# AgentMaker/PAPC

Measured on AMD Instinct MI355X. Metric: point-clouds/sec (fwd+bwd) PointNet++SSG B=32 N=4096, higher is better.
Workload: dtype f32

## Files before the change

papc_amd/csrc/capi.hip:

```cpp
#include <stdarg.h>
#include <string.h>

#include <mutex>
#include <vector>

#include "common.h"

#define GEMM_PARTS_DEFAULT 768

namespace papc {

static thread_local char g_err[512] = "";

void set_error(const char *fmt, ...)
{
    va_list ap;
    va_start(ap, fmt);
    vsnprintf(g_err, sizeof(g_err), fmt, ap);
    va_end(ap);
}

int check_launch(const char *what)
{
    hipError_t e = hipGetLastError();
    if (e != hipSuccess) {
        set_error("%s: %s", what, hipGetErrorString(e));
        return PAPC_E_LAUNCH;
    }
    return PAPC_OK;
}

struct KnobDef { const char *name; int def, lo, hi; };
static const KnobDef g_knob_defs[KNOB_COUNT] = {
    {"PAPC_LG_PARTS", 2048, 1, 8192},
    {"PAPC_DW_F32", 0, 0, 1},
    {"PAPC_DW_DBG", 0, 0, 1},
    {"PAPC_DW_XYZ", 1, 0, 1},
    {"PAPC_PARTS", GEMM_PARTS_DEFAULT, 1, 1024},
    {"PAPC_GEMM_F32", 0, 0, 1},
    {"PAPC_GEMM_WAVES", 0, 0, 8},
    {"PAPC_MAXCAT_WAVES", 8, 4, 8},
    {"PAPC_GEMM_WS", 0, 0, 3},
    {"PAPC_GEMM_OCC", 0, 0, 1},
    {"PAPC_GEMM_DBG", 0, 0, 1},
    {"PAPC_GEMM_KB", 0, 0, 2},
    {"PAPC_GEMM_MINWG", 192, 1, 4096},
    {"PAPC_GEMM_TL", 0, 0, 1},
    {"PAPC_FPS_THREADS", 0, 0, 1024},
    {"PAPC_FPS_THREADS_SMALL", 0, 0, 1024},
    {"PAPC_STREAM", 1, 0, 1},
    {"PAPC_STREAM_MINTILES", 2048, 1, 1 << 30},
    {"PAPC_STREAM_CK", 0, 0, 8},
    {"PAPC_STREAM_ASM", 1, 0, 1},
    {"PAPC_PFN_MFMA", 1, 0, 1},
    {"PAPC_DW_RS64", 1, 0, 1},
    {"PAPC_DW_ROWS", 1, 0, 1},
    {"PAPC_DW_ROWS_BLOCKS", 4, 1, 16},
    {"PAPC_DW_ROWSX", 1, 0, 1},
    {"PAPC_PG_DBG", 0, 0, 15},
    {"PAPC_PG_NB", 0, 0, 2},
    {"PAPC_PG_NS", 0, 0, 3},
    {"PAPC_STREAM_MAXCAT", 1, 0, 1},
    {"PAPC_MAX_NOSTORE", 1, 0, 1},
    {"PAPC_PFN_FUSED_TAILS", 1, 0, 1},
    {"PAPC_STREAM_NW12", 1, 0, 1},
    {"PAPC_LG_LISTS", 1, 0, 1},
    {"PAPC_FOLD_WAVES", 16, 8, 16},
    {"PAPC_LGL_VARIANT", 0, 0, 3},
    {"PAPC_LG_PP", 1, 0, 1},
    {"PAPC_PG_GROUP", 1, 0, 1},
};
static int g_knobs[KNOB_COUNT];
static int knob_parse(int id, const char *e)
{
    const KnobDef &d = g_knob_defs[id];
    if (!e || !*e) return d.def;
    const int v = atoi(e);
    return (v < d.lo || v > d.hi) ? d.def : v;
}
static const bool g_knobs_loaded = [] {
    for (int i = 0; i < KNOB_COUNT; ++i) g_knobs[i] = knob_parse(i, getenv(g_knob_defs[i].name));
    return true;
}();
int knob(int id) { return g_knobs[id]; }

struct ProfState {
    std::mutex mu;
    unsigned mask = 0;
    std::vector<std::pair<hipEvent_t, hipEvent_t>> pending[PAPC_K_COUNT];
    std::vector<hipEvent_t> pool;
    double total_ms[PAPC_K_COUNT] = {0};
    int64_t launches[PAPC_K_COUNT] = {0};
};
static ProfState g_prof;

static hipEvent_t prof_get_event()
{
    if (!g_prof.pool.empty()) {
        hipEvent_t e = g_prof.pool.back();
        g_prof.pool.pop_back();
        return e;
    }
    hipEvent_t e;
    if (hipEventCreate(&e) != hipSuccess) return nullptr;
    return e;
}

ProfScope::ProfScope(int k, hipStream_t s) : kernel(k), stream(s), on(false), e0(nullptr)
{
    if (!(g_prof.mask & (1u << k))) return;
    std::lock_guard<std::mutex> lk(g_prof.mu);
    e0 = prof_get_event();
    if (!e0) return;
    on = hipEventRecord(e0, stream) == hipSuccess;
}

ProfScope::~ProfScope()
{
    if (!on) return;
    std::lock_guard<std::mutex> lk(g_prof.mu);
    hipEvent_t e1 = prof_get_event();
    if (!e1) return;
    if (hipEventRecord(e1, stream) == hipSuccess) g_prof.pending[kernel].push_back({e0, e1});
}

static void prof_drain(int k)
{
    for (auto &pr : g_prof.pending[k]) {
        float ms = 0.f;
        if (hipEventSynchronize(pr.second) == hipSuccess && hipEventElapsedTime(&ms, pr.first, pr.second) == hipSuccess) {
            g_prof.total_ms[k] += ms;
            g_prof.launches[k] += 1;
        }
        g_prof.pool.push_back(pr.first);
        g_prof.pool.push_back(pr.second);
    }
    g_prof.pending[k].clear();
}

}

extern "C" {

int papc_version(void) { return 600;  }

int papc_abi_version(void) { return PAPC_ABI_VERSION; }

int64_t papc_abi_sizeof(const char *struct_name)
{
    if (!struct_name) return -1;
#define PAPC_SIZEOF(T) if (strcmp(struct_name, #T) == 0) return (int64_t)sizeof(T);
    PAPC_SIZEOF(papc_group_src)
    PAPC_SIZEOF(papc_point_lists)
    PAPC_SIZEOF(papc_group_max)
    PAPC_SIZEOF(papc_bwd_dy)
    PAPC_SIZEOF(papc_scatter_dst)
    PAPC_SIZEOF(papc_bwd_red)
    PAPC_SIZEOF(papc_reduce_job)
    PAPC_SIZEOF(papc_fold_job)
    PAPC_SIZEOF(papc_fold_list)
    PAPC_SIZEOF(papc_sa_desc)
    PAPC_SIZEOF(papc_sa_layer)
    PAPC_SIZEOF(papc_compact_src)
    PAPC_SIZEOF(papc_sa_io)
    PAPC_SIZEOF(papc_sa_plan)
    PAPC_SIZEOF(papc_sa_grads)
    PAPC_SIZEOF(papc_pfn_desc)
    PAPC_SIZEOF(papc_pfn_io)
    PAPC_SIZEOF(papc_head_fc_layer)
    PAPC_SIZEOF(papc_head_bwd_job)
    PAPC_SIZEOF(papc_pg_wjob)
    PAPC_SIZEOF(papc_pg_prep)
    PAPC_SIZEOF(papc_pg_gemm)
    PAPC_SIZEOF(papc_pg_fold_job)
    PAPC_SIZEOF(papc_copy_job)
#undef PAPC_SIZEOF
    return -1;
}

const char *papc_last_error_string(void) { return papc::g_err; }

int papc_knob_set(const char *name, int value)
{
    PAPC_REQUIRE(name, PAPC_E_INVALID, "papc_knob_set: null name");
    for (int i = 0; i < papc::KNOB_COUNT; ++i)
        if (!strcmp(name, papc::g_knob_defs[i].name)) {
            PAPC_REQUIRE(value >= papc::g_knob_defs[i].lo && value <= papc::g_knob_defs[i].hi, PAPC_E_INVALID,
                         "papc_knob_set: %s = %d outside [%d, %d]", name, value, papc::g_knob_defs[i].lo, papc::g_knob_defs[i].hi);
            papc::g_knobs[i] = value;
            return PAPC_OK;
        }
    papc::set_error("papc_knob_set: unknown knob %s", name);
    return PAPC_E_INVALID;
}

int papc_knob_get(const char *name, int *value)
{
    PAPC_REQUIRE(name && value, PAPC_E_INVALID, "papc_knob_get: null argument");
    for (int i = 0; i < papc::KNOB_COUNT; ++i)
        if (!strcmp(name, papc::g_knob_defs[i].name)) { *value = papc::g_knobs[i]; return PAPC_OK; }
    papc::set_error("papc_knob_get: unknown knob %s", name);
    return PAPC_E_INVALID;
}

int papc_prof_enable(unsigned mask)
{
    std::lock_guard<std::mutex> lk(papc::g_prof.mu);
    papc::g_prof.mask = mask;
    return PAPC_OK;
}

int papc_prof_reset(void)
{
    std::lock_guard<std::mutex> lk(papc::g_prof.mu);
    for (int k = 0; k < PAPC_K_COUNT; ++k) {
        papc::prof_drain(k);
        papc::g_prof.total_ms[k] = 0;
        papc::g_prof.launches[k] = 0;
    }
    return PAPC_OK;
}

int papc_prof_read(int kernel, double *total_ms, int64_t *launches)
// ... 11 lines not shown
```

papc_amd/csrc/common.h:

```cpp
#pragma once
#include <hip/hip_runtime.h>
#include <stdint.h>
#include <stdio.h>
#include <stdlib.h>
#include <string.h>
#include <algorithm>

#include "papc_hip.h"

namespace papc {

void set_error(const char *fmt, ...);
int check_launch(const char *what);

#define PAPC_REQUIRE(cond, code, ...)      \
    do {                                   \
        if (!(cond)) {                     \
            papc::set_error(__VA_ARGS__);  \
            return (code);                 \
        }                                  \
    } while (0)

enum Knob {
    KNOB_LG_PARTS, KNOB_DW_F32, KNOB_DW_DBG, KNOB_DW_XYZ, KNOB_PARTS, KNOB_GEMM_F32, KNOB_GEMM_WAVES, KNOB_MAXCAT_WAVES,
    KNOB_GEMM_WS, KNOB_GEMM_OCC, KNOB_GEMM_DBG, KNOB_GEMM_KB, KNOB_GEMM_MINWG, KNOB_GEMM_TL, KNOB_FPS_THREADS,
    KNOB_FPS_THREADS_SMALL, KNOB_STREAM, KNOB_STREAM_MINTILES, KNOB_STREAM_CK, KNOB_STREAM_ASM, KNOB_PFN_MFMA, KNOB_DW_RS64, KNOB_DW_ROWS, KNOB_DW_ROWS_BLOCKS, KNOB_DW_ROWSX, KNOB_PG_DBG, KNOB_PG_NB, KNOB_PG_NS, KNOB_STREAM_MAXCAT, KNOB_MAX_NOSTORE, KNOB_PFN_FUSED_TAILS, KNOB_STREAM_NW12, KNOB_LG_LISTS, KNOB_FOLD_WAVES, KNOB_LGL_VARIANT, KNOB_LG_PP, KNOB_PG_GROUP, KNOB_COUNT
};
int knob(int id);

struct ProfScope {
    int kernel;
    hipStream_t stream;
    bool on;
    hipEvent_t e0;
    ProfScope(int kernel, hipStream_t stream);
    ~ProfScope();
};

static inline hipStream_t as_stream(papc_stream_t s) { return reinterpret_cast<hipStream_t>(s); }

static inline int64_t cdiv(int64_t a, int64_t b) { return (a + b - 1) / b; }
static inline bool aligned16(const void *p) { return (reinterpret_cast<uintptr_t>(p) & 15) == 0; }

#define PAPC_DPP(v, ctrl, rmask) __builtin_amdgcn_update_dpp((int)(v), (int)(v), (ctrl), (rmask), 0xF, false)

__device__ __forceinline__ float wave_sum_f32_to_lane63(float v)
{
    float t;
    t = __int_as_float(PAPC_DPP(__float_as_int(v), 0xB1, 0xF));  v += t;
    t = __int_as_float(PAPC_DPP(__float_as_int(v), 0x4E, 0xF));  v += t;
    t = __int_as_float(PAPC_DPP(__float_as_int(v), 0x124, 0xF)); v += t;
    t = __int_as_float(PAPC_DPP(__float_as_int(v), 0x128, 0xF)); v += t;
    t = __int_as_float(__builtin_amdgcn_update_dpp(0, __float_as_int(v), 0x142, 0xA, 0xF, false)); v += t;
    t = __int_as_float(__builtin_amdgcn_update_dpp(0, __float_as_int(v), 0x143, 0xC, 0xF, false)); v += t;
    return v;
}

__device__ __forceinline__ float half_sum_f32(float v)
{
    float t;
    t = __int_as_float(PAPC_DPP(__float_as_int(v), 0xB1, 0xF));  v += t;
    t = __int_as_float(PAPC_DPP(__float_as_int(v), 0x4E, 0xF));  v += t;
    t = __int_as_float(PAPC_DPP(__float_as_int(v), 0x124, 0xF)); v += t;
    t = __int_as_float(PAPC_DPP(__float_as_int(v), 0x128, 0xF)); v += t;
    t = __int_as_float(__builtin_amdgcn_update_dpp(0, __float_as_int(v), 0x142, 0xA, 0xF, false)); v += t;
    return v;
}

__device__ __forceinline__ float readlane63_f32(float v)
{
    return __int_as_float(__builtin_amdgcn_readlane(__float_as_int(v), 63));
}


#define PAPC_DPPF(v, ctrl, rmask) __int_as_float(__builtin_amdgcn_update_dpp(__float_as_int(v), __float_as_int(v), (ctrl), (rmask), 0xF, false))
#define PAPC_DPPU(v, ctrl, rmask) ((unsigned)__builtin_amdgcn_update_dpp((int)(v), (int)(v), (ctrl), (rmask), 0xF, false))

__device__ __forceinline__ float row_max_f32(float v)
{
    v = fmaxf(v, PAPC_DPPF(v, 0xB1, 0xF));
    v = fmaxf(v, PAPC_DPPF(v, 0x4E, 0xF));
    v = fmaxf(v, PAPC_DPPF(v, 0x124, 0xF));
    v = fmaxf(v, PAPC_DPPF(v, 0x128, 0xF));
    return v;
}
__device__ __forceinline__ unsigned row_min_u32(unsigned v)
{
    unsigned t;
    t = PAPC_DPPU(v, 0xB1, 0xF);  v = t < v ? t : v;
    t = PAPC_DPPU(v, 0x4E, 0xF);  v = t < v ? t : v;
    t = PAPC_DPPU(v, 0x124, 0xF); v = t < v ? t : v;
    t = PAPC_DPPU(v, 0x128, 0xF); v = t < v ? t : v;
    return v;
}
__device__ __forceinline__ float wave_max_f32_to_lane63(float v)
{
    v = row_max_f32(v);
    v = fmaxf(v, PAPC_DPPF(v, 0x142, 0xA));
    v = fmaxf(v, PAPC_DPPF(v, 0x143, 0xC));
    return v;
}
__device__ __forceinline__ unsigned wave_min_u32_to_lane63(unsigned v)
{
    unsigned t;
    v = row_min_u32(v);
    t = PAPC_DPPU(v, 0x142, 0xA); v = t < v ? t : v;
    t = PAPC_DPPU(v, 0x143, 0xC); v = t < v ? t : v;
    return v;
}
#define PAPC_DPP_STEP(op, v, ctrl) asm volatile("s_nop 1\n\t" op " %0, %0, %0 " ctrl : "+v"(v))
__device__ __forceinline__ unsigned row_max_u32_fused(unsigned v)
{
    PAPC_DPP_STEP("v_max_u32_dpp", v, "quad_perm:[1,0,3,2] row_mask:0xf bank_mask:0xf");
    PAPC_DPP_STEP("v_max_u32_dpp", v, "quad_perm:[2,3,0,1] row_mask:0xf bank_mask:0xf");
    PAPC_DPP_STEP("v_max_u32_dpp", v, "row_ror:4 row_mask:0xf bank_mask:0xf");
    PAPC_DPP_STEP("v_max_u32_dpp", v, "row_ror:8 row_mask:0xf bank_mask:0xf");
    return v;
}
__device__ __forceinline__ unsigned row_min_u32_fused(unsigned v)
{
    PAPC_DPP_STEP("v_min_u32_dpp", v, "quad_perm:[1,0,3,2] row_mask:0xf bank_mask:0xf");
    PAPC_DPP_STEP("v_min_u32_dpp", v, "quad_perm:[2,3,0,1] row_mask:0xf bank_mask:0xf");
    PAPC_DPP_STEP("v_min_u32_dpp", v, "row_ror:4 row_mask:0xf bank_mask:0xf");
    PAPC_DPP_STEP("v_min_u32_dpp", v, "row_ror:8 row_mask:0xf bank_mask:0xf");
    return v;
}
__device__ __forceinline__ unsigned wave_max_u32_fused_to_lane63(unsigned v)
{
    v = row_max_u32_fused(v);
    PAPC_DPP_STEP("v_max_u32_dpp", v, "row_bcast:15 row_mask:0xa bank_mask:0xf");
    PAPC_DPP_STEP("v_max_u32_dpp", v, "row_bcast:31 row_mask:0xc bank_mask:0xf");
    asm volatile("s_nop 1" ::"v"(v));
    return v;
}
__device__ __forceinline__ unsigned wave_min_u32_fused_to_lane63(unsigned v)
{
    v = row_min_u32_fused(v);
    PAPC_DPP_STEP("v_min_u32_dpp", v, "row_bcast:15 row_mask:0xa bank_mask:0xf");
    PAPC_DPP_STEP("v_min_u32_dpp", v, "row_bcast:31 row_mask:0xc bank_mask:0xf");
    asm volatile("s_nop 1" ::"v"(v));
    return v;
}
__device__ __forceinline__ unsigned readlane63_u32(unsigned v) { return (unsigned)__builtin_amdgcn_readlane((int)v, 63); }
__device__ __forceinline__ float readlane0_f32(float v) { return __int_as_float(__builtin_amdgcn_readlane(__float_as_int(v), 0)); }
__device__ __forceinline__ unsigned readlane0_u32(unsigned v) { return (unsigned)__builtin_amdgcn_readlane((int)v, 0); }

__device__ __forceinline__ void lds_barrier()
{
    asm volatile("s_waitcnt lgkmcnt(0)\n\ts_barrier" ::: "memory");
}

__device__ __forceinline__ float relu_np(float t) { return !(t <= 0.f) ? t : 0.f; }
__device__ __forceinline__ int lane_id() { return (int)(threadIdx.x & 63); }

}
```

papc_amd/csrc/smallm.hip:

```cpp
#include "fold.h"
#include "mlp_loaders.h"

namespace papc {

enum { PG_EPI_STORE = 0, PG_EPI_FWD = 1, PG_EPI_FWD_GMAX = 2, PG_EPI_RED = 3 };
enum { PG_PREP_PLAIN = 0, PG_PREP_CONCAT = 1, PG_PREP_BNRELU = 2, PG_PREP_DY_DENSE = 3, PG_PREP_DY_MAX = 4 };

__host__ __device__ static inline int64_t ru64(int64_t a, int64_t b) { return (a + b - 1) / b * b; }

__device__ __forceinline__ void store_planes8(char *frag0, int slot, const float (&v)[8])
{
    bf16x8 pl[3];
    split8(v, pl);
    *reinterpret_cast<uint4 *>(frag0 + slot * 16) = __builtin_bit_cast(uint4, pl[0]);
    *reinterpret_cast<uint4 *>(frag0 + 1024 + slot * 16) = __builtin_bit_cast(uint4, pl[1]);
    *reinterpret_cast<uint4 *>(frag0 + 2048 + slot * 16) = __builtin_bit_cast(uint4, pl[2]);
}

struct WJob {
    const float *src; int64_t sr, sc;
    int R, K;
    char *dst;
};
struct WJobs {
// ... 168 lines not shown
#pragma unroll
                for (int i = 0; i < 8; ++i) e[i] = dy_elem(d[i], e[i], cs[0][kl + i], cs[1][kl + i], cs[2][kl + i], cs[3][kl + i], cs[4][kl + i], cs[5][kl + i]);
            }
#pragma unroll
            for (int i = 0; i < 8; ++i) v[j][i] = (mok && kok) ? e[i] : 0.f;
        }
    }
    if (p.P) {
#pragma unroll
        for (int j = 0; j < 2; ++j) store_planes8(p.P + ((int64_t)mb * p.KBp + cb * 2 + j) * 3072, lane, v[j]);
    }
    if (p.PT) {
#pragma unroll
        for (int j = 0; j < 2; ++j)
#pragma unroll
            for (int i = 0; i < 8; ++i) tile[wv][r_in][16 * j + 8 * h + i] = v[j][i];
        __syncthreads();
#pragma unroll
        for (int j = 0; j < 2; ++j) {
            float u[8];
#pragma unroll
            for (int i = 0; i < 8; ++i) u[i] = tile[wv][16 * j + 8 * h + i][r_in];
            store_planes8(p.PT + ((int64_t)cb * p.KBt + mb * 2 + j) * 3072, lane, u);
        }
    }
}

struct PgArgs {
    const char *a, *b; int KB;
    int nst;
    int R1, R2;
    float *c; int64_t ldc, zstride;
    const float *bias;
    float *stats;
    float *gmax, *gmin; int32_t *amax, *amin;
    const float *y_prev, *mean, *invstd, *scale, *shift;
    int dbg;
    int g1, g2;
};

__device__ __forceinline__ void glds16(const char *g, unsigned lds_addr)
{
    unsigned keep;
    asm volatile("s_mov_b32 %0, m0\n\ts_mov_b32 m0, %2\n\ts_nop 0\n\tglobal_load_lds_dwordx4 %1, off\n\ts_mov_b32 m0, %0"
                 : "=&s"(keep)
                 : "v"(g), "s"(lds_addr)
                 : "memory");
}
template <int N>
__device__ __forceinline__ void pg_wait_barrier()
{
    asm volatile("s_waitcnt vmcnt(%0) lgkmcnt(0)\n\ts_barrier" ::"n"(N) : "memory");
}

template <int EPI, int NB, bool FULL>
__device__ __forceinline__ void pg_epilogue(const PgArgs &p, floatx16 (&acc)[2][NB], char *smem, int lane, int wr, int wc, int bi, int bj, int bz)
{
    const int cl = lane & 31, h = lane >> 5;
    constexpr bool FWD = (EPI == PG_EPI_FWD || EPI == PG_EPI_FWD_GMAX);
    constexpr bool SUMS = FWD || EPI == PG_EPI_RED;
    float *rs = reinterpret_cast<float *>(smem);
    if (SUMS) __syncthreads();
    const int it0 = 2 * wr * 32 + h * 4;
    const int ldc = (int)p.ldc;
#pragma unroll
    for (int ib = 0; ib < NB; ++ib) {
        const int jt = (wc * NB + ib) * 32 + cl;
        const int j = bj * (NB * 64) + jt;
        const bool jok = FULL || j < p.R2;
        const int jj = jok ? j : 0;
        float *cp = p.c + (int64_t)bz * p.zstride + (int64_t)(bi * 128 + it0) * p.ldc + jj;
        float bias = 0.f, sc = 0.f, sh = 0.f, mu = 0.f, is = 0.f;
        if (FWD && p.bias) bias = p.bias[jj];
        if (EPI == PG_EPI_RED) { sc = p.scale[jj]; sh = p.shift[jj]; mu = p.mean[jj]; is = p.invstd[jj]; }
        float yp[2][16];
        if (EPI == PG_EPI_RED) {
            const float *yq = p.y_prev + (int64_t)(bi * 128 + it0) * p.ldc + jj;
#pragma unroll
            for (int ia = 0; ia < 2; ++ia)
#pragma unroll
                for (int r = 0; r < 16; ++r) {
                    const int ro = ia * 32 + (r >> 2) * 8 + (r & 3);
                    yp[ia][r] = (FULL || (jok && bi * 128 + it0 + ro < p.R1)) ? yq[ro * ldc] : 0.f;
                }
        }
        if (FWD) {
#pragma unroll
            for (int ia = 0; ia < 2; ++ia)
#pragma unroll
                for (int r = 0; r < 16; ++r) acc[ia][ib][r] += bias;
        }
#pragma unroll
        for (int ia = 0; ia < 2; ++ia)
#pragma unroll
            for (int r = 0; r < 16; ++r) {
                const int ro = ia * 32 + (r >> 2) * 8 + (r & 3);
                if (FULL) cp[ro * ldc] = acc[ia][ib][r];
                else if (jok && bi * 128 + it0 + ro < p.R1) cp[ro * ldc] = acc[ia][ib][r];
            }
        if (!SUMS) continue;
        float s1 = 0.f, s2 = 0.f, mx = -INFINITY, mn = INFINITY;
        int amx = 0, amn = 0;
#pragma unroll
        for (int ia = 0; ia < 2; ++ia)
#pragma unroll
            for (int r = 0; r < 16; ++r) {
                const int ro = ia * 32 + (r >> 2) * 8 + (r & 3);
                const bool ok = FULL || (jok && bi * 128 + it0 + ro < p.R1);
                const float v = acc[ia][ib][r];
                if (FWD) {
                    s1 += ok ? v : 0.f;
                    s2 = ok ? fmaf(v, v, s2) : s2;
                    if (EPI == PG_EPI_FWD_GMAX) {
                        if (v > mx) { mx = v; amx = it0 + ro; }
                        if (v < mn) { mn = v; amn = it0 + ro; }
                    }
                } else {
                    const float pv = (ok && fmaf(sc, yp[ia][r], sh) > 0.f) ? v : 0.f;
                    s1 += pv;
                    s2 = fmaf(pv, (yp[ia][r] - mu) * is, s2);
                }
            }
        s1 += __shfl_xor(s1, 32); s2 += __shfl_xor(s2, 32);
        if (EPI == PG_EPI_FWD_GMAX) {
            const float omx = __shfl_xor(mx, 32), omn = __shfl_xor(mn, 32);
            const int oamx = __shfl_xor(amx, 32), oamn = __shfl_xor(amn, 32);
            if (omx > mx || (omx == mx && oamx < amx)) { mx = omx; amx = oamx; }
            if (omn < mn || (omn == mn && oamn < amn)) { mn = omn; amn = oamn; }
        }
        if (wr == 1 && h == 0) {
            float *q = rs + jt * 6;
            q[0] = s1; q[1] = s2;
            if (EPI == PG_EPI_FWD_GMAX) { q[2] = mx; q[3] = __int_as_float(amx); q[4] = mn; q[5] = __int_as_float(amn); }
        }
        __syncthreads();
        if (wr == 0 && h == 0 && jok) {
            const float *q = rs + jt * 6;
            p.stats[((int64_t)bi * 2 + 0) * p.R2 + j] = s1 + q[0];
            p.stats[((int64_t)bi * 2 + 1) * p.R2 + j] = s2 + q[1];
            if (EPI == PG_EPI_FWD_GMAX) {
                const float omx = q[2], omn = q[4];
                if (omx > mx) { mx = omx; amx = __float_as_int(q[3]); }
                if (omn < mn) { mn = omn; amn = __float_as_int(q[5]); }
                p.gmax[(int64_t)bi * p.R2 + j] = mx; p.amax[(int64_t)bi * p.R2 + j] = amx;
                p.gmin[(int64_t)bi * p.R2 + j] = mn; p.amin[(int64_t)bi * p.R2 + j] = amn;
            }
        }
    }
}

template <int NB>
constexpr int pg_stage_bytes() { return (4 + 2 * NB) * 6 * 1024; }

template <int EPI, int NB, int NS>
__device__ __forceinline__ void pg_gemm_wg(const PgArgs &p, int t, const int nwg, char *smem)
{
    constexpr int STAGE = pg_stage_bytes<NB>();
    constexpr int NLW = (4 + 2 * NB) * 6 / 4;
    const int lane = threadIdx.x & 63;
    const int w = __builtin_amdgcn_readfirstlane((int)(threadIdx.x >> 6));
    const int wr = w >> 1, wc = w & 1;
    if ((nwg & 7) == 0) t = (t & 7) * (nwg >> 3) + (t >> 3);
    const int tiles = p.g1 * p.g2;
    const int bz = t / tiles;
    t -= bz * tiles;
    const int bi = t / p.g2, bj = t - bi * p.g2;
    const int nst = p.nst;
    const int64_t st0 = (int64_t)bz * nst;
    const unsigned lds0 = (unsigned)(uintptr_t)smem;

    const char *ga = p.a + (((int64_t)bi * 4 + w) * p.KB + st0 * 2) * 3072 + lane * 16;
    const char *gb;
    unsigned sa = (unsigned)(w * 6) * 1024, sbq;
    if (NB == 2) {
        gb = p.b + (((int64_t)bj * 4 + w) * p.KB + st0 * 2) * 3072 + lane * 16;
        sbq = (unsigned)((4 + w) * 6) * 1024;
    } else {
        gb = p.b + (((int64_t)bj * 2 + (w >> 1)) * p.KB + st0 * 2) * 3072 + (w & 1) * 3072 + lane * 16;
        sbq = (unsigned)((4 + (w >> 1)) * 6 + (w & 1) * 3) * 1024;
    }
    auto issue = [&](int s, int buf) {
        const unsigned base = lds0 + (unsigned)buf * STAGE;
        const char *a = ga + (int64_t)s * 6144, *b = gb + (int64_t)s * 6144;
#pragma unroll
        for (int q = 0; q < 6; ++q) glds16(a + q * 1024, __builtin_amdgcn_readfirstlane(base + sa + q * 1024));
#pragma unroll
        for (int q = 0; q < (NB == 2 ? 6 : 3); ++q) glds16(b + q * 1024, __builtin_amdgcn_readfirstlane(base + sbq + q * 1024));
    };

    floatx16 acc[2][NB];
#pragma unroll
    for (int ia = 0; ia < 2; ++ia)
#pragma unroll
        for (int ib = 0; ib < NB; ++ib)
#pragma unroll
            for (int r = 0; r < 16; ++r) acc[ia][ib][r] = 0.f;

    if (!(p.dbg & 2)) {
        issue(0, 0);
        if (NS == 3 && nst > 1) issue(1, 1);
    }
    int buf = 0;
    for (int s = 0; s < nst; ++s) {
        if (NS == 3 && s + 1 < nst) pg_wait_barrier<NLW>();
        else pg_wait_barrier<0>();
        if (s + NS - 1 < nst && !(p.dbg & 2)) issue(s + NS - 1, buf == 0 ? NS - 1 : buf - 1);
        const char *sb = smem + buf * STAGE + lane * 16;
#pragma unroll
        for (int kbl = 0; kbl < 2; ++kbl) {
            if (p.dbg & 4) continue;
            bf16x8 af[2][3], bq[NB][3];
#pragma unroll
            for (int ia = 0; ia < 2; ++ia)
#pragma unroll
                for (int pl = 0; pl < 3; ++pl) af[ia][pl] = *reinterpret_cast<const bf16x8 *>(sb + ((2 * wr + ia) * 6 + kbl * 3 + pl) * 1024);
#pragma unroll
            for (int ib = 0; ib < NB; ++ib)
#pragma unroll
                for (int pl = 0; pl < 3; ++pl) bq[ib][pl] = *reinterpret_cast<const bf16x8 *>(sb + ((4 + wc * NB + ib) * 6 + kbl * 3 + pl) * 1024);
            if (p.dbg & 1) {
#pragma unroll
                for (int ia = 0; ia < 2; ++ia)
#pragma unroll
                    for (int pl = 0; pl < 3; ++pl) asm volatile("" ::"v"(af[ia][pl]));
#pragma unroll
                for (int ib = 0; ib < NB; ++ib)
#pragma unroll
                    for (int pl = 0; pl < 3; ++pl) asm volatile("" ::"v"(bq[ib][pl]));
                continue;
            }
#pragma unroll
            for (int t = 0; t < 6; ++t)
#pragma unroll
                for (int ia = 0; ia < 2; ++ia)
#pragma unroll
                    for (int ib = 0; ib < NB; ++ib)
                        acc[ia][ib] = __builtin_amdgcn_mfma_f32_32x32x16_bf16(af[ia][BF16X3_PA[t]], bq[ib][BF16X3_PB[t]], acc[ia][ib], 0, 0, 0);
        }
        buf = buf == NS - 1 ? 0 : buf + 1;
    }

    if (p.dbg & 8) return;
    const bool full = bi * 128 + 128 <= p.R1 && (bj + 1) * (NB * 64) <= p.R2;
    if (full) pg_epilogue<EPI, NB, true>(p, acc, smem, lane, wr, wc, bi, bj, bz);
    else pg_epilogue<EPI, NB, false>(p, acc, smem, lane, wr, wc, bi, bj, bz);
}

template <int EPI, int NB, int NS>
__global__ __launch_bounds__(256, 1) void pg_gemm_kernel(PgArgs p)
{
    __shared__ __attribute__((aligned(1024))) char smem[NS * pg_stage_bytes<NB>()];
    pg_gemm_wg<EPI, NB, NS>(p, blockIdx.x, gridDim.x, smem);
}

template <int EPI0, int EPI1>
__global__ __launch_bounds__(256, 1) void pg_gemm_group_kernel(PgArgs p0, PgArgs p1, int n0)
{
    __shared__ __attribute__((aligned(1024))) char smem[2 * pg_stage_bytes<1>()];
    const int t = blockIdx.x;
    if (t < n0) pg_gemm_wg<EPI0, 1, 2>(p0, t, n0, smem);
    else pg_gemm_wg<EPI1, 1, 2>(p1, t - n0, (int)gridDim.x - n0, smem);
}

__global__ __launch_bounds__(256) void pg_final_kernel(const float *__restrict__ stats, int parts, int64_t M, int C, const float *__restrict__ gamma,
                                                       const float *__restrict__ beta, float eps, float momentum, float *mean, float *invstd,
                                                       float *scale, float *shift, float *rmean, float *rvar, float *__restrict__ gmax,
                                                       const float *__restrict__ gmin, const int32_t *__restrict__ amax,
                                                       const int32_t *__restrict__ amin, int64_t G, float *__restrict__ out, int32_t *__restrict__ argmax,
                                                       int tpg, float *__restrict__ ysel)
{
    __shared__ double rd[2][4][64];
    __shared__ float cs[2][64];
    const int cl = threadIdx.x & 63, gl = threadIdx.x >> 6;
    const int c = blockIdx.x * 64 + cl;
    const bool cok = c < C;
    double s1 = 0.0, s2 = 0.0;
    if (cok) for (int t = gl; t < parts; t += 4) { s1 += (double)stats[(int64_t)t * 2 * C + c]; s2 += (double)stats[((int64_t)t * 2 + 1) * C + c]; }
    rd[0][gl][cl] = s1; rd[1][gl][cl] = s2;
    __syncthreads();
    if (gl == 0) {
        s1 = (rd[0][0][cl] + rd[0][1][cl]) + (rd[0][2][cl] + rd[0][3][cl]);
        s2 = (rd[1][0][cl] + rd[1][1][cl]) + (rd[1][2][cl] + rd[1][3][cl]);
        float sc = 0.f, sh = 0.f;
        if (cok) {
            const double mu = s1 / (double)M;
            double var = s2 / (double)M - mu * mu;
            if (var < 0.0) var = 0.0;
            const double is = 1.0 / sqrt(var + (double)eps);
            const double scd = (gamma ? (double)gamma[c] : 1.0) * is;
            sc = (float)scd;
            sh = (float)((beta ? (double)beta[c] : 0.0) - mu * scd);
            mean[c] = (float)mu; invstd[c] = (float)is; scale[c] = sc; shift[c] = sh;
            if (rmean) rmean[c] = momentum * rmean[c] + (1.f - momentum) * (float)mu;
            if (rvar) rvar[c] = momentum * rvar[c] + (1.f - momentum) * (float)var;
        }
        cs[0][cl] = sc; cs[1][cl] = sh;
    }
    __syncthreads();
    if (!cok) return;
    const float sc = cs[0][cl], sh = cs[1][cl];
    const bool up = sc >= 0.f;
    if (tpg > 1) {
        const float *gsel = up ? gmax : gmin;
        const int32_t *asel = up ? amax : amin;
        for (int64_t g = gl; g < G; g += 4) {
            float best = up ? -INFINITY : INFINITY;
            int arg = 0;
            for (int t0 = 0; t0 < tpg; t0 += 8) {
                float v[8];
                int a[8];
#pragma unroll
                for (int j = 0; j < 8; ++j) {
                    const int t = t0 + j < tpg ? t0 + j : t0;
                    const int64_t e = (g * tpg + t) * C + c;
                    v[j] = gsel[e]; a[j] = asel[e];
                }
#pragma unroll
                for (int j = 0; j < 8; ++j)
                    if (t0 + j < tpg && (up ? v[j] > best : v[j] < best)) { best = v[j]; arg = (t0 + j) * 128 + a[j]; }
            }
            out[g * C + c] = relu_np(fmaf(sc, best, sh));
            ysel[g * C + c] = best;
            argmax[g * C + c] = arg;
        }
        return;
    }
    for (int64_t g = gl; g < G; g += 4) {
        const int64_t e = g * C + c;
        const float sel = up ? gmax[e] : gmin[e];
        out[e] = relu_np(fmaf(sc, sel, sh));
        gmax[e] = sel;
        argmax[e] = up ? amax[e] : amin[e];
    }
}

struct FoldJob {
    const float *part; int nsplit; int64_t stride, n; float *out; int accumulate;
};
struct FoldJobs {
    FoldJob j[8];
};
__global__ __launch_bounds__(256) void pg_fold_kernel(FoldJobs jobs)
{
    const FoldJob jb = jobs.j[blockIdx.y];
    const int64_t n4 = jb.n >> 2;
    for (int64_t e = (int64_t)blockIdx.x * 256 + threadIdx.x; e < n4; e += (int64_t)gridDim.x * 256) {
        float4 s = fold_in_order<1, FOLD_FROM_FIRST, float4>(jb.part, jb.stride, jb.nsplit, e * 4);
        float4 *o = reinterpret_cast<float4 *>(jb.out + e * 4);
        if (jb.accumulate) s = fold_add(s, *o);
        *o = s;
    }
    if (blockIdx.x == 0) {
        for (int64_t e = (n4 << 2) + threadIdx.x; e < jb.n; e += 256) {
            const float s = fold_in_order<1, FOLD_FROM_FIRST, float>(jb.part, jb.stride, jb.nsplit, e);
            jb.out[e] = jb.accumulate ? jb.out[e] + s : s;
        }
    }
}

}

using namespace papc;

extern "C" {

size_t papc_pg_planes_bytes(int64_t R, int64_t K)
{
    if (R < 1 || K < 1) return 0;
    return (size_t)(ru64(R, 128) * ru64(K, 32) * 6);
}

int papc_pg_prep_weights_f32(const papc_pg_wjob *jobs, int count, papc_stream_t stream)
{
    PAPC_REQUIRE(jobs && count >= 1 && count <= 8, PAPC_E_INVALID, "papc_pg_prep_weights_f32: 1..8 jobs");
    WJobs wj;
    memset(&wj, 0, sizeof(wj));
    int64_t most = 0;
    for (int i = 0; i < count; ++i) {
        PAPC_REQUIRE(jobs[i].src && jobs[i].planes && jobs[i].R >= 1 && jobs[i].K >= 1, PAPC_E_INVALID, "papc_pg_prep_weights_f32: bad job %d", i);
        PAPC_REQUIRE(aligned16(jobs[i].planes), PAPC_E_INVALID, "papc_pg_prep_weights_f32: planes must be 16-byte aligned");
        wj.j[i].src = jobs[i].src; wj.j[i].sr = jobs[i].row_stride; wj.j[i].sc = jobs[i].col_stride; wj.j[i].R = jobs[i].R; wj.j[i].K = jobs[i].K;
        wj.j[i].dst = reinterpret_cast<char *>(jobs[i].planes);
        most = std::max<int64_t>(most, (ru64(jobs[i].R, 32) / 32) * (ru64(jobs[i].K, 32) / 16));
    }
    hipStream_t st = as_stream(stream);
    ProfScope prof(PAPC_K_MISC, st);
    hipLaunchKernelGGL(pg_prep_w_kernel, dim3((unsigned)std::min<int64_t>(cdiv(most, 4), 512), (unsigned)count), dim3(256), 0, st, wj);
    return check_launch("papc_pg_prep_weights_f32");
}

int papc_pg_prep_rows_f32(const papc_pg_prep *a, papc_stream_t stream)
{
    PAPC_REQUIRE(a, PAPC_E_INVALID, "papc_pg_prep_rows_f32: null args");
    PAPC_REQUIRE(a->M >= 1 && a->M < (1ll << 31) && a->C >= 1, PAPC_E_INVALID, "papc_pg_prep_rows_f32: bad sizes");
    PAPC_REQUIRE(a->planes || a->planes_t, PAPC_E_INVALID, "papc_pg_prep_rows_f32: no output");
    PAPC_REQUIRE((!a->planes || aligned16(a->planes)) && (!a->planes_t || aligned16(a->planes_t)), PAPC_E_INVALID, "papc_pg_prep_rows_f32: planes must be 16-byte aligned");
    PAPC_REQUIRE(!a->planes_t || a->M % 32 == 0, PAPC_E_UNSUPPORTED, "papc_pg_prep_rows_f32: transposed planes need M %% 32 == 0");
    PrepArgs p;
    memset(&p, 0, sizeof(p));
    p.M = a->M; p.C = a->C;
    p.P = reinterpret_cast<char *>(a->planes); p.KBp = (int)(ru64(a->C, 32) / 16);
    p.PT = reinterpret_cast<char *>(a->planes_t); p.KBt = (int)(ru64(a->M, 32) / 16);
    const int mode = a->mode;
    if (mode == PG_PREP_CONCAT) {
        PAPC_REQUIRE(a->xyz && a->N >= 1 && a->M % a->N == 0 && a->D >= 0 && a->C == a->D + 3 && (a->D == 0 || a->feats), PAPC_E_INVALID,
                     "papc_pg_prep_rows_f32: CONCAT needs xyz, feats [M, D], C == D + 3, N | M");
        p.xyz = a->xyz; p.sb = a->sb; p.sn = a->sn; p.sc = a->sc; p.feats = a->feats; p.N = a->N; p.D = a->D; p.xyz_first = a->xyz_first;
    } else {
        PAPC_REQUIRE(mode == PG_PREP_PLAIN || mode == PG_PREP_BNRELU || mode == PG_PREP_DY_DENSE || mode == PG_PREP_DY_MAX, PAPC_E_INVALID,
                     "papc_pg_prep_rows_f32: bad mode %d", mode);
        PAPC_REQUIRE(a->x && a->ldx >= a->C, PAPC_E_INVALID, "papc_pg_prep_rows_f32: x null or ldx < C");
        PAPC_REQUIRE(a->C % 8 == 0 && a->ldx % 4 == 0 && aligned16(a->x), PAPC_E_UNSUPPORTED, "papc_pg_prep_rows_f32: needs C %% 8 == 0 and 16-byte aligned rows");
        p.x = a->x; p.ldx = a->ldx;
    }
    if (mode == PG_PREP_BNRELU) {
        PAPC_REQUIRE(a->stats && a->parts >= 1 && a->mean && a->invstd && a->scale && a->shift, PAPC_E_INVALID, "papc_pg_prep_rows_f32: BNRELU needs stats and the four constant vectors");
        p.stats = a->stats; p.parts = a->parts; p.gamma = a->gamma; p.beta = a->beta; p.eps = a->eps; p.momentum = a->momentum;
        p.rmean = a->running_mean; p.rvar = a->running_var;
    }
    if (mode == PG_PREP_DY_DENSE || mode == PG_PREP_DY_MAX) {
        PAPC_REQUIRE(a->mean && a->invstd && a->scale && a->shift, PAPC_E_INVALID, "papc_pg_prep_rows_f32: DY needs the layer's BN constants");
        PAPC_REQUIRE(a->ldx == a->C, PAPC_E_INVALID, "papc_pg_prep_rows_f32: DY needs dense y (ldx == C)");
        if (mode == PG_PREP_DY_DENSE) {
            PAPC_REQUIRE(a->dz && aligned16(a->dz) && a->red && a->red_parts >= 1, PAPC_E_INVALID, "papc_pg_prep_rows_f32: DY_DENSE needs dz and the red partials");
        } else {
            PAPC_REQUIRE(a->gout && a->argmax && a->K >= 1 && a->M % a->K == 0 && aligned16(a->gout) && aligned16(a->argmax), PAPC_E_INVALID,
                         "papc_pg_prep_rows_f32: DY_MAX needs gout / argmax [M/K, C] and K | M");
            PAPC_REQUIRE(a->red || a->ysel, PAPC_E_INVALID, "papc_pg_prep_rows_f32: DY_MAX needs red partials or ysel");
        }
        p.dz = a->dz; p.gout = a->gout; p.ysel = a->ysel; p.argmax = a->argmax; p.K = a->K > 0 ? a->K : 1;
        p.red = a->red; p.red_parts = a->red_parts; p.dgamma = a->dgamma; p.dbeta = a->dbeta; p.accumulate = a->accumulate;
    }
    p.mean = a->mean; p.invstd = a->invstd; p.scale = a->scale; p.shift = a->shift;
    hipStream_t st = as_stream(stream);
    ProfScope prof(PAPC_K_MISC, st);
    const dim3 grid((unsigned)(ru64(a->C, 32) / 32), (unsigned)(ru64(a->M, 128) / 128));
    switch (mode) {
    case PG_PREP_PLAIN: hipLaunchKernelGGL(pg_prep_kernel<PG_PREP_PLAIN>, grid, dim3(256), 0, st, p); break;
    case PG_PREP_CONCAT: hipLaunchKernelGGL(pg_prep_kernel<PG_PREP_CONCAT>, grid, dim3(256), 0, st, p); break;
    case PG_PREP_BNRELU: hipLaunchKernelGGL(pg_prep_kernel<PG_PREP_BNRELU>, grid, dim3(256), 0, st, p); break;
    case PG_PREP_DY_DENSE: hipLaunchKernelGGL(pg_prep_kernel<PG_PREP_DY_DENSE>, grid, dim3(256), 0, st, p); break;
    default: hipLaunchKernelGGL(pg_prep_kernel<PG_PREP_DY_MAX>, grid, dim3(256), 0, st, p); break;
    }
    return check_launch("papc_pg_prep_rows_f32");
}

}

namespace papc {

static int pg_args(const papc_pg_gemm *g, PgArgs &p, int *split_out)
{
    PAPC_REQUIRE(g && g->a && g->b && g->c, PAPC_E_INVALID, "papc_pg_gemm_f32: null pointer");
    PAPC_REQUIRE(g->R1 >= 1 && g->R2 >= 1 && g->K >= 1 && g->ldc >= g->R2, PAPC_E_INVALID, "papc_pg_gemm_f32: bad sizes");
    PAPC_REQUIRE(aligned16(g->a) && aligned16(g->b), PAPC_E_INVALID, "papc_pg_gemm_f32: planes must be 16-byte aligned");
    const int nst_all = (int)(ru64(g->K, 32) / 32);
    const int split = g->split >= 1 ? g->split : 1;
    PAPC_REQUIRE(nst_all % split == 0, PAPC_E_INVALID, "papc_pg_gemm_f32: split %d does not divide the %d k32 stages", split, nst_all);
    PAPC_REQUIRE(split == 1 || g->epi == PG_EPI_STORE, PAPC_E_INVALID, "papc_pg_gemm_f32: split K only with the plain store epilogue");
    memset(&p, 0, sizeof(p));
    p.a = reinterpret_cast<const char *>(g->a); p.b = reinterpret_cast<const char *>(g->b); p.KB = nst_all * 2; p.nst = nst_all / split;
    p.R1 = g->R1; p.R2 = g->R2; p.c = g->c; p.ldc = g->ldc; p.zstride = g->split_stride;
    p.bias = g->bias; p.stats = g->stats; p.dbg = knob(KNOB_PG_DBG);
    const int epi = g->epi;
    PAPC_REQUIRE(epi >= PG_EPI_STORE && epi <= PG_EPI_RED, PAPC_E_INVALID, "papc_pg_gemm_f32: bad epilogue %d", epi);
    if (epi == PG_EPI_FWD || epi == PG_EPI_FWD_GMAX || epi == PG_EPI_RED) PAPC_REQUIRE(g->stats, PAPC_E_INVALID, "papc_pg_gemm_f32: this epilogue needs stats");
    if (epi == PG_EPI_FWD_GMAX) {
        PAPC_REQUIRE(g->gmax && g->gmin && g->amax && g->amin && g->R1 % 128 == 0, PAPC_E_INVALID, "papc_pg_gemm_f32: GMAX needs its four arrays and whole 128-row groups");
        p.gmax = g->gmax; p.gmin = g->gmin; p.amax = g->amax; p.amin = g->amin;
    }
    if (epi == PG_EPI_RED) {
        PAPC_REQUIRE(g->y_prev && g->mean && g->invstd && g->scale && g->shift && g->ldc == g->R2, PAPC_E_INVALID, "papc_pg_gemm_f32: RED needs the layer below (dense)");
        p.y_prev = g->y_prev; p.mean = g->mean; p.invstd = g->invstd; p.scale = g->scale; p.shift = g->shift;
    }
    *split_out = split;
    return PAPC_OK;
}

}

extern "C" {

int papc_pg_gemm_f32(const papc_pg_gemm *g, papc_stream_t stream)
{
    PgArgs p;
    int split = 1;
    const int rc = pg_args(g, p, &split);
    if (rc != PAPC_OK) return rc;
    const int epi = g->epi;
    hipStream_t st = as_stream(stream);
    ProfScope prof(g->family >= 0 && g->family < PAPC_K_COUNT ? g->family : PAPC_K_MISC, st);
    const int64_t t1 = cdiv(g->R1, 128);
    int nb = knob(KNOB_PG_NB), ns = knob(KNOB_PG_NS);
    if (nb == 0) nb = (g->R2 > 64 && t1 * cdiv(g->R2, 128) * split >= 200) ? 2 : 1;
    if (g->R2 <= 64) nb = 1;
    if (ns == 0) ns = 2;
    p.g1 = (int)t1; p.g2 = (int)cdiv(g->R2, nb == 2 ? 128 : 64);
    const dim3 grid((unsigned)(p.g1 * p.g2 * split));
#define PG_GO(E)                                                                                      \
    do {                                                                                              \
        if (nb == 2 && ns == 3) hipLaunchKernelGGL((pg_gemm_kernel<E, 2, 3>), grid, dim3(256), 0, st, p);      \
        else if (nb == 2) hipLaunchKernelGGL((pg_gemm_kernel<E, 2, 2>), grid, dim3(256), 0, st, p);            \
        else if (ns == 3) hipLaunchKernelGGL((pg_gemm_kernel<E, 1, 3>), grid, dim3(256), 0, st, p);            \
        else hipLaunchKernelGGL((pg_gemm_kernel<E, 1, 2>), grid, dim3(256), 0, st, p);                         \
    } while (0)
    switch (epi) {
    case PG_EPI_STORE: PG_GO(PG_EPI_STORE); break;
    case PG_EPI_FWD: PG_GO(PG_EPI_FWD); break;
    case PG_EPI_FWD_GMAX: PG_GO(PG_EPI_FWD_GMAX); break;
    default: PG_GO(PG_EPI_RED); break;
    }
#undef PG_GO
    return check_launch("papc_pg_gemm_f32");
}

int papc_pg_gemm_group_f32(const papc_pg_gemm *g, int count, papc_stream_t stream)
{
    PAPC_REQUIRE(g && (count == 1 || count == 2), PAPC_E_INVALID, "papc_pg_gemm_group_f32: 1 or 2 products");
    PgArgs p[2];
    int split[2] = {1, 1};
    for (int i = 0; i < count; ++i) {
        const int rc = pg_args(&g[i], p[i], &split[i]);
        if (rc != PAPC_OK) return rc;
        PAPC_REQUIRE(g[i].epi == PG_EPI_STORE || g[i].epi == PG_EPI_RED, PAPC_E_UNSUPPORTED,
                     "papc_pg_gemm_group_f32: product %d: only the store and dX (RED) epilogues share a launch", i);
    }
    PAPC_REQUIRE(count == 1 || g[0].epi != PG_EPI_RED || g[1].epi != PG_EPI_RED, PAPC_E_UNSUPPORTED, "papc_pg_gemm_group_f32: at most one dX (RED) product per launch");
    if (count == 1 || !knob(KNOB_PG_GROUP) || knob(KNOB_PG_NB) == 2 || knob(KNOB_PG_NS) == 3) {
        for (int i = 0; i < count; ++i) {
            const int rc = papc_pg_gemm_f32(&g[i], stream);
            if (rc != PAPC_OK) return rc;
        }
        return PAPC_OK;
    }
    int n[2];
    for (int i = 0; i < 2; ++i) {
        p[i].g1 = (int)cdiv(g[i].R1, 128); p[i].g2 = (int)cdiv(g[i].R2, 64);
        n[i] = p[i].g1 * p[i].g2 * split[i];
    }
    const int f = p[1].nst > p[0].nst ? 1 : 0, s = 1 - f;
    const int e0 = g[f].epi, e1 = g[s].epi;
    hipStream_t st = as_stream(stream);
    ProfScope prof(g[f].family >= 0 && g[f].family < PAPC_K_COUNT ? g[f].family : PAPC_K_MISC, st);
    const dim3 grid((unsigned)(n[0] + n[1]));
    if (e0 == PG_EPI_RED) hipLaunchKernelGGL((pg_gemm_group_kernel<PG_EPI_RED, PG_EPI_STORE>), grid, dim3(256), 0, st, p[f], p[s], n[f]);
    else if (e1 == PG_EPI_RED) hipLaunchKernelGGL((pg_gemm_group_kernel<PG_EPI_STORE, PG_EPI_RED>), grid, dim3(256), 0, st, p[f], p[s], n[f]);
    else hipLaunchKernelGGL((pg_gemm_group_kernel<PG_EPI_STORE, PG_EPI_STORE>), grid, dim3(256), 0, st, p[f], p[s], n[f]);
    return check_launch("papc_pg_gemm_group_f32");
}

int papc_pg_final_f32(const float *stats, int parts, int64_t M, int C, const float *gamma, const float *beta, float eps, float momentum,
                      float *mean, float *invstd, float *scale, float *shift, float *running_mean, float *running_var, float *gmax,
                      const float *gmin, const int32_t *amax, const int32_t *amin, int64_t G, float *out, int32_t *argmax, papc_stream_t stream)
{
    PAPC_REQUIRE(stats && mean && invstd && scale && shift && gmax && gmin && amax && amin && out && argmax, PAPC_E_INVALID, "papc_pg_final_f32: null pointer");
    PAPC_REQUIRE(parts >= 1 && M >= 1 && C >= 1 && G >= 1, PAPC_E_INVALID, "papc_pg_final_f32: bad sizes");
    hipStream_t st = as_stream(stream);
    ProfScope prof(PAPC_K_BN_RELU_MAX, st);
    hipLaunchKernelGGL(pg_final_kernel, dim3((unsigned)cdiv(C, 64)), dim3(256), 0, st, stats, parts, M, C, gamma, beta, eps, momentum, mean, invstd,
                       scale, shift, running_mean, running_var, gmax, gmin, amax, amin, G, out, argmax, 1, (float *)nullptr);
    return check_launch("papc_pg_final_f32");
}

int papc_pg_final_groups_f32(const float *stats, int parts, int64_t M, int C, const float *gamma, const float *beta, float eps, float momentum,
                             float *mean, float *invstd, float *scale, float *shift, float *running_mean, float *running_var, const float *gmax,
                             const float *gmin, const int32_t *amax, const int32_t *amin, int64_t G, int tiles_per_group, float *out, int32_t *argmax,
                             float *ysel, papc_stream_t stream)
{
    PAPC_REQUIRE(stats && mean && invstd && scale && shift && gmax && gmin && amax && amin && out && argmax && ysel, PAPC_E_INVALID, "papc_pg_final_groups_f32: null pointer");
    PAPC_REQUIRE(parts >= 1 && M >= 1 && C >= 1 && G >= 1 && tiles_per_group >= 2, PAPC_E_INVALID, "papc_pg_final_groups_f32: bad sizes (tiles_per_group >= 2; 1 is papc_pg_final_f32)");
    hipStream_t st = as_stream(stream);
    ProfScope prof(PAPC_K_BN_RELU_MAX, st);
    hipLaunchKernelGGL(pg_final_kernel, dim3((unsigned)cdiv(C, 64)), dim3(256), 0, st, stats, parts, M, C, gamma, beta, eps, momentum, mean, invstd,
                       scale, shift, running_mean, running_var, const_cast<float *>(gmax), gmin, amax, amin, G, out, argmax, tiles_per_group, ysel);
    return check_launch("papc_pg_final_groups_f32");
}

int papc_pg_fold_f32(const papc_pg_fold_job *jobs, int count, papc_stream_t stream)
{
    PAPC_REQUIRE(jobs && count >= 1 && count <= 8, PAPC_E_INVALID, "papc_pg_fold_f32: 1..8 jobs");
    FoldJobs fj;
    memset(&fj, 0, sizeof(fj));
    int64_t most = 0;
    for (int i = 0; i < count; ++i) {
        PAPC_REQUIRE(jobs[i].partial && jobs[i].out && jobs[i].nsplit >= 1 && jobs[i].n >= 1, PAPC_E_INVALID, "papc_pg_fold_f32: bad job %d", i);
        PAPC_REQUIRE(aligned16(jobs[i].partial) && aligned16(jobs[i].out) && jobs[i].stride % 4 == 0, PAPC_E_INVALID, "papc_pg_fold_f32: 16-byte alignment");
        fj.j[i].part = jobs[i].partial; fj.j[i].nsplit = jobs[i].nsplit; fj.j[i].stride = jobs[i].stride; fj.j[i].n = jobs[i].n;
        fj.j[i].out = jobs[i].out; fj.j[i].accumulate = jobs[i].accumulate;
        most = std::max<int64_t>(most, jobs[i].n);
    }
    hipStream_t st = as_stream(stream);
    ProfScope prof(PAPC_K_BWD_DW, st);
    hipLaunchKernelGGL(pg_fold_kernel, dim3((unsigned)std::max<int64_t>(1, std::min<int64_t>(cdiv(most, 1024), 1024)), (unsigned)count), dim3(256), 0, st, fj);
    return check_launch("papc_pg_fold_f32");
}

}
```

Before: 20940.

## Add four-slot k16 LDS ring pipeline for pg GEMM main loop

Adds a new main-loop path for the pg GEMM kernels. It splits each two-stage LDS buffer into four half-size slots and keeps up to four k16 sub-blocks of global-to-LDS loads in flight, with counted waits. It also double-buffers register fragment reads and uses sched_group_barrier to interleave LDS reads with MFMAs. The aim is to hide global load latency and LDS read latency behind matrix math, at the cost of more complex wait logic and higher register pressure. It is enabled by default through a new knob for both single and grouped launches when using two stages.

Result: faster. 21410, median of 6 (+2.3%).

```diff
diff --git a/papc_amd/csrc/capi.hip b/papc_amd/csrc/capi.hip
--- a/papc_amd/csrc/capi.hip
+++ b/papc_amd/csrc/capi.hip
@@ -69,6 +69,7 @@
     {"PAPC_LGL_VARIANT", 0, 0, 3},
     {"PAPC_LG_PP", 1, 0, 1},
     {"PAPC_PG_GROUP", 1, 0, 1},
+    {"PAPC_PG_PIPE", 1, 0, 1},
 };
 static int g_knobs[KNOB_COUNT];
 static int knob_parse(int id, const char *e)
diff --git a/papc_amd/csrc/common.h b/papc_amd/csrc/common.h
--- a/papc_amd/csrc/common.h
+++ b/papc_amd/csrc/common.h
@@ -24,7 +24,7 @@
 enum Knob {
     KNOB_LG_PARTS, KNOB_DW_F32, KNOB_DW_DBG, KNOB_DW_XYZ, KNOB_PARTS, KNOB_GEMM_F32, KNOB_GEMM_WAVES, KNOB_MAXCAT_WAVES,
     KNOB_GEMM_WS, KNOB_GEMM_OCC, KNOB_GEMM_DBG, KNOB_GEMM_KB, KNOB_GEMM_MINWG, KNOB_GEMM_TL, KNOB_FPS_THREADS,
-    KNOB_FPS_THREADS_SMALL, KNOB_STREAM, KNOB_STREAM_MINTILES, KNOB_STREAM_CK, KNOB_STREAM_ASM, KNOB_PFN_MFMA, KNOB_DW_RS64, KNOB_DW_ROWS, KNOB_DW_ROWS_BLOCKS, KNOB_DW_ROWSX, KNOB_PG_DBG, KNOB_PG_NB, KNOB_PG_NS, KNOB_STREAM_MAXCAT, KNOB_MAX_NOSTORE, KNOB_PFN_FUSED_TAILS, KNOB_STREAM_NW12, KNOB_LG_LISTS, KNOB_FOLD_WAVES, KNOB_LGL_VARIANT, KNOB_LG_PP, KNOB_PG_GROUP, KNOB_COUNT
+    KNOB_FPS_THREADS_SMALL, KNOB_STREAM, KNOB_STREAM_MINTILES, KNOB_STREAM_CK, KNOB_STREAM_ASM, KNOB_PFN_MFMA, KNOB_DW_RS64, KNOB_DW_ROWS, KNOB_DW_ROWS_BLOCKS, KNOB_DW_ROWSX, KNOB_PG_DBG, KNOB_PG_NB, KNOB_PG_NS, KNOB_STREAM_MAXCAT, KNOB_MAX_NOSTORE, KNOB_PFN_FUSED_TAILS, KNOB_STREAM_NW12, KNOB_LG_LISTS, KNOB_FOLD_WAVES, KNOB_LGL_VARIANT, KNOB_LG_PP, KNOB_PG_GROUP, KNOB_PG_PIPE, KNOB_COUNT
 };
 int knob(int id);
 
diff --git a/papc_amd/csrc/smallm.hip b/papc_amd/csrc/smallm.hip
--- a/papc_amd/csrc/smallm.hip
+++ b/papc_amd/csrc/smallm.hip
@@ -344,7 +344,101 @@
 template <int NB>
 constexpr int pg_stage_bytes() { return (4 + 2 * NB) * 6 * 1024; }
 
-template <int EPI, int NB, int NS>
+template <int NB>
+constexpr int pg_slot_bytes() { return (4 + 2 * NB) * 3 * 1024; }
+
+template <int L>
+__device__ __forceinline__ void pg_wait_barrier_ahead(int ahead)
+{
+    if (ahead >= 3) pg_wait_barrier<3 * L>();
+    else if (ahead == 2) pg_wait_barrier<2 * L>();
+    else if (ahead == 1) pg_wait_barrier<L>();
+    else pg_wait_barrier<0>();
+}
+
+template <int NB>
+__device__ __forceinline__ void pg_ring_k16(const PgArgs &p, floatx16 (&acc)[2][NB], char *smem, int lane, int w, int bi, int bj, int64_t st0, int nblk)
+{
+    constexpr int SLOT = pg_slot_bytes<NB>();
+    const int wr = w >> 1, wc = w & 1;
+    const unsigned lds0 = (unsigned)(uintptr_t)smem;
+    const int64_t kb0 = st0 * 2;
+    const char *ga = p.a + (((int64_t)bi * 4 + w) * p.KB + kb0) * 3072 + lane * 16;
+    const unsigned sa = (unsigned)(w * 3) * 1024;
+    const int f0 = NB == 2 ? 0 : (w < 2 ? 2 * w : 2 + w), f1 = f0 + 1;
+    const char *gb0, *gb1;
+    unsigned sbq;
+    if (NB == 2) {
+        gb0 = p.b + (((int64_t)bj * 4 + w) * p.KB + kb0) * 3072 + lane * 16;
+        gb1 = gb0;
+        sbq = (unsigned)((4 + w) * 3) * 1024;
+    } else {
+        gb0 = p.b + (((int64_t)bj * 2 + f0 / 3) * p.KB + kb0) * 3072 + (f0 % 3) * 1024 + lane * 16;
+        gb1 = p.b + (((int64_t)bj * 2 + f1 / 3) * p.KB + kb0) * 3072 + (f1 % 3) * 1024 + lane * 16;
+        sbq = (unsigned)(4 * 3 + f0) * 1024;
+    }
+    auto issue = [&](int s, int slot) {
+        const unsigned base = lds0 + (unsigned)slot * SLOT;
+        const int64_t o = (int64_t)s * 3072;
+#pragma unroll
+        for (int q = 0; q < 3; ++q) glds16(ga + o + q * 1024, __builtin_amdgcn_readfirstlane(base + sa + q * 1024));
+        if (NB == 2) {
+#pragma unroll
+            for (int q = 0; q < 3; ++q) glds16(gb0 + o + q * 1024, __builtin_amdgcn_readfirstlane(base + sbq + q * 1024));
+        } else {
+            glds16(gb0 + o, __builtin_amdgcn_readfirstlane(base + sbq));
+            if (w < 2) glds16(gb1 + o, __builtin_amdgcn_readfirstlane(base + sbq + 1024));
+        }
+    };
+    auto wait = [&](int ahead) {
+        if (NB == 2) pg_wait_barrier_ahead<6>(ahead);
+        else if (w < 2) pg_wait_barrier_ahead<5>(ahead);
+        else pg_wait_barrier_ahead<4>(ahead);
+    };
+    bf16x8 af[2][2][3], bq[2][NB][3];
+    auto read = [&](bf16x8 (&a)[2][3], bf16x8 (&b)[NB][3], int slot) {
+        const char *sb = smem + slot * SLOT + lane * 16;
+#pragma unroll
+        for (int ia = 0; ia < 2; ++ia)
+#pragma unroll
+            for (int pl = 0; pl < 3; ++pl) a[ia][pl] = *reinterpret_cast<const bf16x8 *>(sb + ((2 * wr + ia) * 3 + pl) * 1024);
+#pragma unroll
+        for (int ib = 0; ib < NB; ++ib)
+#pragma unroll
+            for (int pl = 0; pl < 3; ++pl) b[ib][pl] = *reinterpret_cast<const bf16x8 *>(sb + ((4 + wc * NB + ib) * 3 + pl) * 1024);
+    };
+
+    const int n0 = nblk < 4 ? nblk : 4;
+    for (int s = 0; s < n0; ++s) issue(s, s);
+    wait(n0 - 1);
+    read(af[0], bq[0], 0);
+    for (int s2 = 0; s2 < nblk; s2 += 2) {
+#pragma unroll
+        for (int u = 0; u < 2; ++u) {
+            const int s = s2 + u;
+            const int left = nblk - 2 - s;
+            wait(left < 0 ? 0 : left > 2 ? 2 : left);
+            if (s + 4 < nblk) issue(s + 4, s & 3);
+            read(af[u ^ 1], bq[u ^ 1], (s + 1) & 3);
+#pragma unroll
+            for (int t = 0; t < 6; ++t)
+#pragma unroll
+                for (int ia = 0; ia < 2; ++ia)
+#pragma unroll
+                    for (int ib = 0; ib < NB; ++ib)
+                        acc[ia][ib] = __builtin_amdgcn_mfma_f32_32x32x16_bf16(af[u][ia][BF16X3_PA[t]], bq[u][ib][BF16X3_PB[t]], acc[ia][ib], 0, 0, 0);
+#pragma unroll
+            for (int i = 0; i < 6 + 3 * NB; ++i) {
+                __builtin_amdgcn_sched_group_barrier(0x008, 1, 0);
+                __builtin_amdgcn_sched_group_barrier(0x100, 1, 0);
+            }
+            __builtin_amdgcn_sched_group_barrier(0x008, 12 * NB - (6 + 3 * NB), 0);
+        }
+    }
+}
+
+
+template <int EPI, int NB, int NS, bool PIPE>
 __device__ __forceinline__ void pg_gemm_wg(const PgArgs &p, int t, const int nwg, char *smem)
 {
     constexpr int STAGE = pg_stage_bytes<NB>();
@@ -388,6 +482,17 @@
 #pragma unroll
             for (int r = 0; r < 16; ++r) acc[ia][ib][r] = 0.f;
 
+    auto epilogue = [&] {
+        const bool full = bi * 128 + 128 <= p.R1 && (bj + 1) * (NB * 64) <= p.R2;
+        if (full) pg_epilogue<EPI, NB, true>(p, acc, smem, lane, wr, wc, bi, bj, bz);
+        else pg_epilogue<EPI, NB, false>(p, acc, smem, lane, wr, wc, bi, bj, bz);
+    };
+    if constexpr (PIPE) {
+        pg_ring_k16<NB>(p, acc, smem, lane, w, bi, bj, st0, 2 * nst);
+        epilogue();
+        return;
+    }
+
     if (!(p.dbg & 2)) {
         issue(0, 0);
         if (NS == 3 && nst > 1) issue(1, 1);
@@ -433,25 +538,24 @@
     }
 
     if (p.dbg & 8) return;
-    const bool full = bi * 128 + 128 <= p.R1 && (bj + 1) * (NB * 64) <= p.R2;
-    if (full) pg_epilogue<EPI, NB, true>(p, acc, smem, lane, wr, wc, bi, bj, bz);
-    else pg_epilogue<EPI, NB, false>(p, acc, smem, lane, wr, wc, bi, bj, bz);
-}
-
-template <int EPI, int NB, int NS>
+    epilogue();
+}
+
+template <int EPI, int NB, int NS, bool PIPE>
 __global__ __launch_bounds__(256, 1) void pg_gemm_kernel(PgArgs p)
 {
+    static_assert(!PIPE || (NS == 2 && 4 * pg_slot_bytes<NB>() == NS * pg_stage_bytes<NB>()), "the k16 ring lives in the two-stage footprint");
     __shared__ __attribute__((aligned(1024))) char smem[NS * pg_stage_bytes<NB>()];
-    pg_gemm_wg<EPI, NB, NS>(p, blockIdx.x, gridDim.x, smem);
-}
-
-template <int EPI0, int EPI1>
+    pg_gemm_wg<EPI, NB, NS, PIPE>(p, blockIdx.x, gridDim.x, smem);
+}
+
+template <int EPI0, int EPI1, bool PIPE>
 __global__ __launch_bounds__(256, 1) void pg_gemm_group_kernel(PgArgs p0, PgArgs p1, int n0)
 {
     __shared__ __attribute__((aligned(1024))) char smem[2 * pg_stage_bytes<1>()];
     const int t = blockIdx.x;
-    if (t < n0) pg_gemm_wg<EPI0, 1, 2>(p0, t, n0, smem);
-    else pg_gemm_wg<EPI1, 1, 2>(p1, t - n0, (int)gridDim.x - n0, smem);
+    if (t < n0) pg_gemm_wg<EPI0, 1, 2, PIPE>(p0, t, n0, smem);
+    else pg_gemm_wg<EPI1, 1, 2, PIPE>(p1, t - n0, (int)gridDim.x - n0, smem);
 }
 
 __global__ __launch_bounds__(256) void pg_final_kernel(const float *__restrict__ stats, int parts, int64_t M, int C, const float *__restrict__ gamma,
@@ -687,14 +791,17 @@
     if (nb == 0) nb = (g->R2 > 64 && t1 * cdiv(g->R2, 128) * split >= 200) ? 2 : 1;
     if (g->R2 <= 64) nb = 1;
     if (ns == 0) ns = 2;
+    const bool pipe = knob(KNOB_PG_PIPE) && ns == 2 && !p.dbg;
     p.g1 = (int)t1; p.g2 = (int)cdiv(g->R2, nb == 2 ? 128 : 64);
     const dim3 grid((unsigned)(p.g1 * p.g2 * split));
 #define PG_GO(E)                                                                                      \
     do {                                                                                              \
-        if (nb == 2 && ns == 3) hipLaunchKernelGGL((pg_gemm_kernel<E, 2, 3>), grid, dim3(256), 0, st, p);      \
-        else if (nb == 2) hipLaunchKernelGGL((pg_gemm_kernel<E, 2, 2>), grid, dim3(256), 0, st, p);            \
-        else if (ns == 3) hipLaunchKernelGGL((pg_gemm_kernel<E, 1, 3>), grid, dim3(256), 0, st, p);            \
-        else hipLaunchKernelGGL((pg_gemm_kernel<E, 1, 2>), grid, dim3(256), 0, st, p);                         \
+        if (nb == 2 && ns == 3) hipLaunchKernelGGL((pg_gemm_kernel<E, 2, 3, false>), grid, dim3(256), 0, st, p);      \
+        else if (nb == 2 && pipe) hipLaunchKernelGGL((pg_gemm_kernel<E, 2, 2, true>), grid, dim3(256), 0, st, p);     \
+        else if (nb == 2) hipLaunchKernelGGL((pg_gemm_kernel<E, 2, 2, false>), grid, dim3(256), 0, st, p);            \
+        else if (ns == 3) hipLaunchKernelGGL((pg_gemm_kernel<E, 1, 3, false>), grid, dim3(256), 0, st, p);            \
+        else if (pipe) hipLaunchKernelGGL((pg_gemm_kernel<E, 1, 2, true>), grid, dim3(256), 0, st, p);                \
+        else hipLaunchKernelGGL((pg_gemm_kernel<E, 1, 2, false>), grid, dim3(256), 0, st, p);                         \
     } while (0)
     switch (epi) {
     case PG_EPI_STORE: PG_GO(PG_EPI_STORE); break;
@@ -735,9 +842,16 @@
     hipStream_t st = as_stream(stream);
     ProfScope prof(g[f].family >= 0 && g[f].family < PAPC_K_COUNT ? g[f].family : PAPC_K_MISC, st);
     const dim3 grid((unsigned)(n[0] + n[1]));
-    if (e0 == PG_EPI_RED) hipLaunchKernelGGL((pg_gemm_group_kernel<PG_EPI_RED, PG_EPI_STORE>), grid, dim3(256), 0, st, p[f], p[s], n[f]);
-    else if (e1 == PG_EPI_RED) hipLaunchKernelGGL((pg_gemm_group_kernel<PG_EPI_STORE, PG_EPI_RED>), grid, dim3(256), 0, st, p[f], p[s], n[f]);
-    else hipLaunchKernelGGL((pg_gemm_group_kernel<PG_EPI_STORE, PG_EPI_STORE>), grid, dim3(256), 0, st, p[f], p[s], n[f]);
+#define PG_GO(E0, E1)                                                                                                              \
+    do {                                                                                                                           \
+        if (pipe) hipLaunchKernelGGL((pg_gemm_group_kernel<E0, E1, true>), grid, dim3(256), 0, st, p[f], p[s], n[f]);              \
+        else hipLaunchKernelGGL((pg_gemm_group_kernel<E0, E1, false>), grid, dim3(256), 0, st, p[f], p[s], n[f]);                  \
+    } while (0)
+    const bool pipe = knob(KNOB_PG_PIPE) && !knob(KNOB_PG_DBG);
+    if (e0 == PG_EPI_RED) PG_GO(PG_EPI_RED, PG_EPI_STORE);
+    else if (e1 == PG_EPI_RED) PG_GO(PG_EPI_STORE, PG_EPI_RED);
+    else PG_GO(PG_EPI_STORE, PG_EPI_STORE);
+#undef PG_GO
     return check_launch("papc_pg_gemm_group_f32");
 }
 
```
